# ZhangYizhao/UltraRE

Measured on AMD Instinct MI355X. Metric: training interactions/sec + unlearn retrain wall-time, ml-1m 5-shard SISA, higher is better.
Workload: dtype f32; 1 GPU; ml1m-shaped synthetic 6040x3416, 896914 train rows, 5-shard SISA (uniform grouping), d=32, batch=30000, SGD-momentum-L2, all shards of a rank side by side; parallelism=shards x1, arch=gfx950:sramecc+:xnack-

## Files before the change

ultrare_amd/csrc/perm_chain.hip:

```cpp
#include "ure_internal.h"
#include "mt_jump_dev.h"

namespace ure {
namespace {

constexpr int kMtN = 624, kMtLag = 227;
constexpr int kDrawBlock = 640;
constexpr int kDrawWide = 623;
constexpr int kDrawRing = 8192;
constexpr int64_t kSegmentedRows = 1 << 21;
constexpr int kFewBuckets = 1024;
constexpr int kMaxBuckets = 16384;
constexpr int kTileBlock = 1024;
constexpr int kTileLoads = 4;
constexpr int kTile = kTileBlock * 4 * kTileLoads;
constexpr int kLinkBlock = 512;
constexpr int kLinkLoads = 8;
constexpr int kStage = 6144;
constexpr int kStage10 = 3072, kStage12 = 12288;
constexpr int kStageHeavy = 16384;
constexpr int kHeavyParts = 8;
constexpr int kResolveBlock = 1024;
constexpr int kResolveRows = 4096;
constexpr unsigned kNone = 0xffffffffu;
constexpr unsigned kGoOn = 0x80000000u;
constexpr int64_t kRecordRows = 1 << 20;
constexpr int kRecordShift = 20;
constexpr int kRecordRangeLog2 = 32 - kRecordShift;

__device__ __forceinline__ void lds_barrier()
{
    __builtin_amdgcn_fence(__ATOMIC_RELEASE, "workgroup", "local");
    __builtin_amdgcn_s_barrier();
    __builtin_amdgcn_fence(__ATOMIC_ACQUIRE, "workgroup", "local");
}

__device__ __forceinline__ unsigned mt_temper(unsigned x)
{
    x ^= x >> 11;
    x ^= (x << 7) & 0x9d2c5680u;
    x ^= (x << 15) & 0xefc60000u;
    x ^= x >> 18;
    return x;
}

__device__ __forceinline__ unsigned swap_target(unsigned j, unsigned word, unsigned n) { return j + mt_temper(word) % (n - j); }

template <bool Rec>
struct swap_fmt;
template <>
struct swap_fmt<false> {
    using type = uint2;
    static __device__ __forceinline__ type make(unsigned j, unsigned q, unsigned) { return make_uint2(j, q); }
    static __device__ __forceinline__ type none() { return make_uint2(0u, 0u); }
    static __device__ __forceinline__ unsigned index(type r) { return r.x; }
    static __device__ __forceinline__ unsigned place(type r, unsigned q0) { return r.y - q0; }
};
template <>
struct swap_fmt<true> {
    using type = unsigned;
    static __device__ __forceinline__ type make(unsigned j, unsigned q, unsigned in_range) { return j | (q & in_range) << kRecordShift; }
    static __device__ __forceinline__ type none() { return 0u; }
    static __device__ __forceinline__ unsigned index(type r) { return r & ((1u << kRecordShift) - 1u); }
    static __device__ __forceinline__ unsigned place(type r, unsigned) { return r >> kRecordShift; }
};

struct perm_view {
    unsigned *t, *H, *minv;
    uint2 *pairs;
    unsigned *totals, *cursors, *bases;
};

__host__ __device__ __forceinline__ int64_t words_per_perm(int64_t n_al, int64_t b_al) { return 5 * n_al + 3 * b_al; }

__device__ __forceinline__ perm_view view_of(unsigned *scratch, int perm, int64_t n_al, int64_t b_al)
{
    unsigned *b = scratch + (size_t)perm * (size_t)words_per_perm(n_al, b_al);
    unsigned *c = b + 5 * n_al;
    return perm_view{b, b + n_al, b + 2 * n_al, reinterpret_cast<uint2 *>(b + 3 * n_al), c, c + b_al, c + 2 * b_al};
}

__device__ __forceinline__ unsigned mt_mix(unsigned a, unsigned b)
{
    const unsigned y = (a & 0x80000000u) | (b & 0x7fffffffu);
    return (y >> 1) ^ ((y & 1u) ? 0x9908b0dfu : 0u);
}

__global__ __launch_bounds__(kDrawBlock) void shuffle_seed_kernel(const ure_perm_t *__restrict__ perms, int n_perms, unsigned *__restrict__ states, int J)
{
    const int perm = blockIdx.x, tid = threadIdx.x;
    if (perm >= n_perms) return;
    unsigned *mine = states + (size_t)perm * J * kMtN;
    for (int k = kMtN + tid; k < J * kMtN; k += kDrawBlock) mine[k] = 0u;
    if (tid == 0) {
        unsigned v = (unsigned)((unsigned long long)perms[perm].seed & 0xffffffffull);
        mine[0] = v;
        for (int j = 1; j < kMtN; ++j) {
            v = 1812433253u * (v ^ (v >> 30)) + (unsigned)j;
            mine[j] = v;
        }
    }
}

__global__ __launch_bounds__(kDrawBlock) void shuffle_words_kernel(const ure_perm_t *__restrict__ perms, int n_perms, unsigned *__restrict__ scratch, int64_t n_al,
                                                                   int64_t b_al, int range_log2, const unsigned *__restrict__ states, int J)
{
    constexpr unsigned M = kDrawRing - 1;
    __shared__ unsigned ring[kDrawRing];
    const int tid = threadIdx.x;
    const int perm = blockIdx.x / J, seg = blockIdx.x % J;
    if (perm >= n_perms) return;
    const int n = perms[perm].n;
    if (n <= 0) return;
    const perm_view P = view_of(scratch, perm, n_al, b_al);
    if (seg == 0) {
        const int n_buckets = (int)((((int64_t)n - 1) >> range_log2) + 1);
        for (int b = tid; b < n_buckets; b += kDrawBlock) {
            P.totals[b] = 0u;
            P.cursors[b] = 0u;
        }
    }
    const int64_t w_lo = (int64_t)seg * jmp::kSegWords;
    const int64_t total_all = (int64_t)n - 1;
    if (w_lo >= total_all) return;
    const int total = (int)min<int64_t>(states ? jmp::kSegWords : total_all, total_all - w_lo);
    if (states) {
        const unsigned *blk = states + ((size_t)perm * J + seg) * kMtN;
        for (int k = tid; k < kMtN; k += kDrawBlock) ring[((unsigned)k - kMtN) & M] = blk[k];
    } else if (tid == 0) {
        unsigned v = (unsigned)((unsigned long long)perms[perm].seed & 0xffffffffull);
        ring[(0u - kMtN) & M] = v;
        for (int j = 1; j < kMtN; ++j) {
            v = 1812433253u * (v ^ (v >> 30)) + (unsigned)j;
            ring[((unsigned)j - kMtN) & M] = v;
        }
    }
    __syncthreads();
    unsigned *out = P.t + w_lo;
#pragma unroll 1
    for (int g0 = 0; g0 < total; g0 += kDrawWide) {
        const unsigned g = (unsigned)(g0 + tid);
        if (tid < kDrawWide && (int)g < total) {
            const bool two = g >= (unsigned)kMtLag, three = g >= 2u * kMtLag;
            const unsigned a0 = ring[(g - kMtN) & M], a1 = ring[(g - kMtN + 1) & M];
            const unsigned b0 = ring[(g - kMtLag - kMtN) & M], b1 = ring[(g - kMtLag - kMtN + 1) & M];
            const unsigned c0 = ring[(g - 2 * kMtLag - kMtN) & M], c1 = ring[(g - 2 * kMtLag - kMtN + 1) & M];
            const unsigned x = ring[(g - (three ? 3u * kMtLag : two ? 2u * kMtLag : (unsigned)kMtLag)) & M];
            const unsigned v = x ^ mt_mix(a0, a1) ^ (two ? mt_mix(b0, b1) : 0u) ^ (three ? mt_mix(c0, c1) : 0u);
            ring[g & M] = v;
            out[g] = v;
        }
        lds_barrier();
    }
}

template <int CAP, bool Rec>
__global__ __launch_bounds__(kTileBlock) void shuffle_targets_kernel(const ure_perm_t *__restrict__ perms, int n_perms, int parts_max, unsigned *__restrict__ scratch,
                                                                      int64_t n_al, int64_t b_al, int range_log2, unsigned *__restrict__ mat)
{
    __shared__ unsigned cnt[CAP];
    const int tid = threadIdx.x;
    const int x8 = blockIdx.x & 7, l = blockIdx.x >> 3;
    const int perm = (l / parts_max) * 8 + x8, part = l % parts_max;
    if (perm >= n_perms) return;
    const int n = perms[perm].n;
    const int64_t j0l = (int64_t)part * kTile;
    if (j0l >= (int64_t)n - 1) return;
    const perm_view P = view_of(scratch, perm, n_al, b_al);
    const int n_buckets = (int)((((int64_t)n - 1) >> range_log2) + 1);
    const unsigned j0 = (unsigned)j0l, j_end = (unsigned)(n - 1);
    const int b_lo = (int)(j0 >> range_log2);
    for (int b = b_lo + tid; b < n_buckets; b += kTileBlock) cnt[b] = 0u;
    __syncthreads();
    uint4 *t4 = reinterpret_cast<uint4 *>(P.t);
    uint4 v[kTileLoads];
#pragma unroll
    for (int u = 0; u < kTileLoads; ++u) {
        const unsigned j = j0 + 4u * (unsigned)(tid + u * kTileBlock);
        v[u] = j < j_end ? t4[j >> 2] : make_uint4(0u, 0u, 0u, 0u);
    }
    auto target = [&](unsigned j, unsigned word) {
        if (j >= j_end) return word;
        const unsigned q = swap_target(j, word, (unsigned)n);
        atomicAdd(&cnt[q >> range_log2], 1u);
        return q;
    };
#pragma unroll
    for (int u = 0; u < kTileLoads; ++u) {
        const unsigned j = j0 + 4u * (unsigned)(tid + u * kTileBlock);
        if (j < j_end) {
            v[u].x = target(j, v[u].x);
            v[u].y = target(j + 1, v[u].y);
            v[u].z = target(j + 2, v[u].z);
            v[u].w = target(j + 3, v[u].w);
            if (!Rec) t4[j >> 2] = v[u];
        }
    }
    __syncthreads();
    if (CAP == kFewBuckets) {
        unsigned *row = mat + ((size_t)perm * parts_max + part) * kFewBuckets;
        for (int b = tid; b < n_buckets; b += kTileBlock) row[b] = b >= b_lo ? cnt[b] : 0u;
        return;
    }
    for (int b = b_lo + tid; b < n_buckets; b += kTileBlock) {
        const unsigned c = cnt[b];
        if (c) atomicAdd(&P.totals[b], c);
    }
}

__device__ __forceinline__ bool place_of(int parts_max, int n_perms, int *perm, int *part)
{
    const int x = blockIdx.x & 7, l = blockIdx.x >> 3;
    *perm = (l / parts_max) * 8 + x;
    *part = l % parts_max;
    return *perm < n_perms;
}

template <int Block>
__device__ __forceinline__ unsigned prefix_in_place(unsigned *v, int n, unsigned *wave_sum, unsigned *carry_word)
{
    const int tid = threadIdx.x, lane = tid & 63, wave = tid >> 6;
    if (tid == 0) *carry_word = 0u;
    __syncthreads();
    for (int base = 0; base < n; base += Block) {
        const int x = base + tid;
        const unsigned c = x < n ? v[x] : 0u;
        unsigned s = c;
#pragma unroll
        for (int d = 1; d < 64; d <<= 1) {
            const unsigned o = __shfl_up(s, d, 64);
            if (lane >= d) s += o;
        }
        if (lane == 63) wave_sum[wave] = s;
        __syncthreads();
        unsigned before = *carry_word;
        for (int k = 0; k < wave; ++k) before += wave_sum[k];
        if (x < n) v[x] = before + s - c;
        __syncthreads();
        if (tid == Block - 1) *carry_word = before + s;
    }
    __syncthreads();
    return *carry_word;
}

template <int CAP, bool Rec>
__global__ __launch_bounds__(kTileBlock) void shuffle_bucket_kernel(const ure_perm_t *__restrict__ perms, int n_perms, int parts_max, unsigned *__restrict__ scratch,
                                                                     int64_t n_al, int64_t b_al, int range_log2, const unsigned *__restrict__ mat)
{
    __shared__ unsigned cur[CAP];
    __shared__ unsigned base[CAP];
    __shared__ unsigned wave_sum[kTileBlock / 64];
    __shared__ unsigned s_carry;
    const int tid = threadIdx.x;
    int perm, part;
    if (!place_of(parts_max, n_perms, &perm, &part)) return;
    const int n = perms[perm].n;
    const int64_t j0l = (int64_t)part * kTile;
    if (j0l >= (int64_t)n - 1) {
        if (!(part == 0 && n == 1)) return;
    }
    const perm_view P = view_of(scratch, perm, n_al, b_al);
    const int n_buckets = (int)((((int64_t)n - 1) >> range_log2) + 1);
    const unsigned j0 = (unsigned)j0l, j_end = (unsigned)(n - 1);
    const int b_lo = (int)(j0 >> range_log2);
    const uint4 *t4 = reinterpret_cast<const uint4 *>(P.t);
    uint4 v[kTileLoads];
#pragma unroll
    for (int u = 0; u < kTileLoads; ++u) {
        const unsigned j = j0 + 4u * (unsigned)(tid + u * kTileBlock);
        v[u] = j < j_end ? t4[j >> 2] : make_uint4(0u, 0u, 0u, 0u);
    }
    if (CAP == kFewBuckets) {
        const int n_tiles = (int)(((int64_t)n - 1 + kTile - 1) / kTile);
        const unsigned *m = mat + (size_t)perm * parts_max * kFewBuckets;
        for (int b = tid; b < n_buckets; b += kTileBlock) {
            unsigned all = 0u, before = 0u;
            constexpr int kAtOnce = 8;
            for (int t0 = 0; t0 < n_tiles; t0 += kAtOnce) {
                unsigned c[kAtOnce];
#pragma unroll
                for (int k = 0; k < kAtOnce; ++k) c[k] = m[(size_t)min(t0 + k, n_tiles - 1) * kFewBuckets + b];
#pragma unroll
                for (int k = 0; k < kAtOnce; ++k) {
                    const unsigned ck = t0 + k < n_tiles ? c[k] : 0u;
                    before += t0 + k < part ? ck : 0u;
                    all += ck;
                }
            }
            base[b] = all;
            cur[b] = before;
            if (part == 0) P.totals[b] = all;
        }
        prefix_in_place<kTileBlock>(base, n_buckets, wave_sum, &s_carry);
        for (int b = tid; b < n_buckets; b += kTileBlock) {
            if (part == 0) P.bases[b] = base[b];
            cur[b] += base[b];
        }
        __syncthreads();
    } else {
        for (int b = tid; b < n_buckets; b += kTileBlock) {
            cur[b] = 0u;
            base[b] = P.totals[b];
        }
        __syncthreads();
#pragma unroll
        for (int u = 0; u < kTileLoads; ++u) {
            const unsigned j = j0 + 4u * (unsigned)(tid + u * kTileBlock);
            if (j < j_end) atomicAdd(&cur[v[u].x >> range_log2], 1u);
            if (j + 1 < j_end) atomicAdd(&cur[v[u].y >> range_log2], 1u);
            if (j + 2 < j_end) atomicAdd(&cur[v[u].z >> range_log2], 1u);
            if (j + 3 < j_end) atomicAdd(&cur[v[u].w >> range_log2], 1u);
        }
        prefix_in_place<kTileBlock>(base, n_buckets, wave_sum, &s_carry);
        if (part == 0)
            for (int b = tid; b < n_buckets; b += kTileBlock) P.bases[b] = base[b];
        for (int b = b_lo + tid; b < n_buckets; b += kTileBlock) {
            const unsigned c = cur[b];
            if (c) cur[b] = base[b] + atomicAdd(&P.cursors[b], c);
        }
        __syncthreads();
    }
    static_assert(!Rec || CAP == kFewBuckets, "records: the count matrix's launches only");
    using fmt = swap_fmt<Rec>;
    typename fmt::type *stretches = reinterpret_cast<typename fmt::type *>(P.pairs);
    const unsigned in_range = (1u << range_log2) - 1u;
    auto put = [&](unsigned j, unsigned w) {
        const unsigned q = Rec ? swap_target(j, w, (unsigned)n) : w;
        stretches[atomicAdd(&cur[q >> range_log2], 1u)] = fmt::make(j, q, in_range);
    };
    __builtin_amdgcn_s_waitcnt(0x0F70);
#pragma unroll
    for (int u = 0; u < kTileLoads; ++u) {
        const unsigned j = j0 + 4u * (unsigned)(tid + u * kTileBlock);
        if (j < j_end) put(j, v[u].x);
        if (j + 1 < j_end) put(j + 1, v[u].y);
        if (j + 2 < j_end) put(j + 2, v[u].z);
        if (j + 3 < j_end) put(j + 3, v[u].w);
    }
}

template <int Block, int Per>
__device__ __forceinline__ unsigned prefix_by_lane(unsigned *v, unsigned *wave_sum)
{
    const int tid = threadIdx.x, lane = tid & 63, wave = tid >> 6;
    unsigned c[Per];
    unsigned mine = 0u;
#pragma unroll
    for (int k = 0; k < Per; ++k) {
        c[k] = v[tid * Per + k];
        mine += c[k];
    }
    unsigned s = mine;
#pragma unroll
    for (int d = 1; d < 64; d <<= 1) {
        const unsigned o = __shfl_up(s, d, 64);
        if (lane >= d) s += o;
    }
    if (lane == 63) wave_sum[wave] = s;
    __syncthreads();
    unsigned before = 0u, total = 0u;
#pragma unroll
    for (int k = 0; k < Block / 64; ++k) {
        const unsigned ws = wave_sum[k];
        if (k < wave) before += ws;
        total += ws;
    }
    unsigned run = before + s - mine;
#pragma unroll
    for (int k = 0; k < Per; ++k) {
        v[tid * Per + k] = run;
        run += c[k];
    }
    __syncthreads();
    return total;
}

template <int RL, int Stage, bool Rec>
__global__ __launch_bounds__(kLinkBlock) void shuffle_link_kernel(const ure_perm_t *__restrict__ perms, int n_perms, int parts_max, unsigned *__restrict__ scratch,
                                                                   int64_t n_al, int64_t b_al, int heavy)
{
    static_assert(!Rec || RL <= kRecordRangeLog2, "a record has 12 bits for the target's place in its range");
    using fmt = swap_fmt<Rec>;
    using swap_t = typename fmt::type;
    constexpr int kRange = 1 << RL, kPer = kRange / kLinkBlock;
    __shared__ unsigned off[kRange];
    __shared__ unsigned stage[Stage];
    __shared__ unsigned wave_sum[kLinkBlock / 64];
    const int tid = threadIdx.x;
    int perm, part;
    if (!place_of(parts_max, n_perms, &perm, &part)) return;
    const int n = perms[perm].n;
    const int64_t q0l = (int64_t)part << RL;
    if (q0l >= n) return;
    const int n_buckets = (int)((((int64_t)n - 1) >> RL) + 1);
    if ((part >= n_buckets - kHeavyParts) != (heavy != 0)) return;
    const unsigned q0 = (unsigned)q0l, q1 = (unsigned)min<int64_t>(n, q0l + kRange);
    const int R = (int)(q1 - q0);
    const perm_view P = view_of(scratch, perm, n_al, b_al);
    const unsigned count = P.totals[part], at = P.bases[part];
    const swap_t *mine = reinterpret_cast<const swap_t *>(P.pairs) + at;
#pragma unroll
    for (int k = 0; k < kPer; ++k) off[k * kLinkBlock + tid] = 0u;
    __syncthreads();
    swap_t first[kLinkLoads];
#pragma unroll
    for (int u = 0; u < kLinkLoads; ++u) {
        const unsigned e = (unsigned)(u * kLinkBlock + tid);
        first[u] = e < count ? mine[e] : fmt::none();
    }
#pragma unroll
    for (int u = 0; u < kLinkLoads; ++u)
        if ((unsigned)(u * kLinkBlock + tid) < count) atomicAdd(&off[fmt::place(first[u], q0)], 1u);
    for (unsigned e0 = kLinkBlock * kLinkLoads; e0 < count; e0 += kLinkBlock * kLinkLoads) {
        swap_t m[kLinkLoads];
#pragma unroll
        for (int u = 0; u < kLinkLoads; ++u) {
            const unsigned e = e0 + (unsigned)(u * kLinkBlock + tid);
            m[u] = mine[min(e, count - 1u)];
        }
#pragma unroll
        for (int u = 0; u < kLinkLoads; ++u)
            if (e0 + (unsigned)(u * kLinkBlock + tid) < count) atomicAdd(&off[fmt::place(m[u], q0)], 1u);
    }
    __syncthreads();
    prefix_by_lane<kLinkBlock, kPer>(off, wave_sum);
    const bool in_lds = count <= (unsigned)Stage;
    unsigned *placed = P.t + at;
    auto place = [&](const swap_t m) {
        const unsigned pos = atomicAdd(&off[fmt::place(m, q0)], 1u);
        if (in_lds)
            stage[pos] = fmt::index(m);
        else
            placed[pos] = fmt::index(m);
    };
#pragma unroll
    for (int u = 0; u < kLinkLoads; ++u)
        if ((unsigned)(u * kLinkBlock + tid) < count) place(first[u]);
    for (unsigned e0 = kLinkBlock * kLinkLoads; e0 < count; e0 += kLinkBlock * kLinkLoads) {
        swap_t m[kLinkLoads];
#pragma unroll
        for (int u = 0; u < kLinkLoads; ++u) {
            const unsigned e = e0 + (unsigned)(u * kLinkBlock + tid);
            m[u] = mine[min(e, count - 1u)];
        }
#pragma unroll
        for (int u = 0; u < kLinkLoads; ++u)
            if (e0 + (unsigned)(u * kLinkBlock + tid) < count) place(m[u]);
    }
    if (in_lds) {
        __syncthreads();
    } else {
        __builtin_amdgcn_fence(__ATOMIC_RELEASE, "workgroup");
        __syncthreads();
        __builtin_amdgcn_fence(__ATOMIC_ACQUIRE, "workgroup");
    }
    const unsigned last = (unsigned)(n - 1);
    for (int b0 = 0; b0 < R; b0 += kLinkBlock) {
        unsigned seg0 = 0u;
        bool staged = in_lds;
        if (!in_lds) {
            seg0 = b0 ? off[b0 - 1] : 0u;
            const unsigned seg1 = off[min(b0 + kLinkBlock, R) - 1];
            staged = seg1 - seg0 <= (unsigned)Stage;
            if (staged)
                for (unsigned i = tid; i < seg1 - seg0; i += kLinkBlock) stage[i] = placed[seg0 + i];
            __syncthreads();
        }
        const int x = b0 + tid;
        if (x < R) {
            const unsigned e1 = off[x], e0 = x ? off[x - 1] : 0u;
            const unsigned q = q0 + (unsigned)x;
            auto walk = [&](auto member) {
                unsigned least = kNone;
                for (unsigned i = e0; i < e1; ++i) {
                    const unsigned a = member(i);
                    least = min(least, a);
                    unsigned succ = kNone;
                    for (unsigned m = e0; m < e1; ++m) {
                        const unsigned o = member(m);
                        if (o > a) succ = min(succ, o);
                    }
                    P.H[a] = succ != kNone ? succ : (a == q ? a : (q == last ? last : (kGoOn | q)));
                }
                P.minv[q] = least;
            };
            if (staged)
                walk([&](unsigned i) { return stage[i - seg0]; });
            else
                walk([&](unsigned i) { return placed[i]; });
        }
        if (!in_lds) __syncthreads();
    }
}

__global__ __launch_bounds__(kResolveBlock) void shuffle_resolve_kernel(const ure_perm_t *__restrict__ perms, int n_perms, int parts_max, unsigned *__restrict__ scratch,
                                                                         int64_t n_al, int64_t b_al, unsigned *__restrict__ broken)
{
    int perm, part;
    if (!place_of(parts_max, n_perms, &perm, &part)) return;
    const int n = perms[perm].n;
    const int64_t lo = (int64_t)part * kResolveRows;
    if (lo >= n) return;
    const perm_view P = view_of(scratch, perm, n_al, b_al);
    const unsigned batch = (unsigned)perms[perm].batch;
    uint16_t *out = perms[perm].tags;
    const unsigned hi = (unsigned)min<int64_t>(n, lo + kResolveRows);
    constexpr int U = 4;
    for (unsigned p0 = (unsigned)lo + threadIdx.x; p0 < hi; p0 += U * kResolveBlock) {
        unsigned v[U], h[U];
#pragma unroll
        for (int u = 0; u < U; ++u) {
            const unsigned p = p0 + (unsigned)(u * kResolveBlock);
            v[u] = p < hi ? P.minv[p] : 0u;
            h[u] = p < hi && p != (unsigned)(n - 1) ? P.H[p] : 0u;
        }
#pragma unroll
        for (int u = 0; u < U; ++u) {
            const unsigned p = p0 + (unsigned)(u * kResolveBlock);
            if (p >= hi) continue;
            unsigned r = v[u];
            if (r == kNone) {
                if (p == (unsigned)(n - 1)) {
                    r = p;
                } else {
                    unsigned at = p;
                    r = h[u];
                    while (r & kGoOn) {
                        const unsigned q = r & ~kGoOn;
                        if (q <= at || q >= (unsigned)(n - 1)) {
                            r = kNone;
                            break;
                        }
                        at = q;
                        r = P.H[q];
                    }
                }
            }
            if (r >= (unsigned)n) {
                *broken = 0xdeadu;
                out[p] = (uint16_t)0xFFFFu;
            } else {
                out[p] = (uint16_t)(r / batch);
            }
        }
    }
}

struct link_launch {
    bool records;
    dim3 grid;
    hipStream_t st;
    const ure_perm_t *perms;
    int n_perms, ranges;
    unsigned *scratch;
    int64_t n_al, b_al;
    int heavy;
    template <int RL, int Stage>
    void go() const
    {
        if constexpr (RL <= kRecordRangeLog2) {
            if (records) {
                hipLaunchKernelGGL((shuffle_link_kernel<RL, Stage, true>), grid, dim3(kLinkBlock), 0, st, perms, n_perms, ranges, scratch, n_al, b_al, heavy);
                return;
            }
        }
        hipLaunchKernelGGL((shuffle_link_kernel<RL, Stage, false>), grid, dim3(kLinkBlock), 0, st, perms, n_perms, ranges, scratch, n_al, b_al, heavy);
    }
};

int range_log2_of(int64_t n_max, int32_t wanted)
{
    if (wanted) return wanted;
    return n_max <= ((int64_t)kMaxBuckets << 10) ? 10 : n_max <= ((int64_t)kMaxBuckets << 11) ? 11 : n_max <= ((int64_t)kMaxBuckets << 12) ? 12 : 14;
}

int64_t buckets_al(int64_t n_max, int rl) { return (((n_max - 1) >> rl) + 1 + 63) / 64 * 64; }

}
}

extern "C" int64_t ure_device_shuffle_tags_flag(int64_t n_max, int32_t n_perms)
{
    if (n_max <= 0 || n_perms <= 0) return 0;
    const int64_t n_al = (n_max + 63) / 64 * 64;
    return ure::words_per_perm(n_al, std::min<int64_t>(ure::kMaxBuckets, ure::buckets_al(n_max, 10))) * (int64_t)n_perms;
}

extern "C" int64_t ure_device_shuffle_tags_scratch(int64_t n_max, int32_t n_perms)
{
    if (n_max <= 0 || n_perms <= 0) return 0;
    const int64_t J = n_max > ure::kSegmentedRows ? (n_max - 1 + ure::jmp::kSegWords - 1) / ure::jmp::kSegWords : 0;
    const int64_t tiles = std::max<int64_t>(1, (n_max - 1 + ure::kTile - 1) / ure::kTile);
    return ure_device_shuffle_tags_flag(n_max, n_perms) + 64 + (int64_t)n_perms * J * ure::kMtN + (int64_t)n_perms * tiles * ure::kFewBuckets;
}

extern "C" int ure_device_shuffle_tags(const ure_perm_t *perms, int32_t n_perms, int64_t n_max, uint32_t *scratch, int64_t scratch_words, int32_t range_log2,
                                       void *stream)
{
    using namespace ure;
    URE_ARG(n_perms >= 0 && n_max >= 0 && (range_log2 == 0 || range_log2 == 10 || range_log2 == 11 || range_log2 == 12 || range_log2 == 14));
    if (n_perms == 0 || n_max == 0) return 0;
    URE_ARG(perms && scratch);
    const int rl = range_log2_of(n_max, range_log2);
    if (((n_max - 1) >> rl) + 1 > kMaxBuckets)
        return fail(-1, "ure_device_shuffle_tags: %lld rows: more than %d ranges of %d targets", (long long)n_max, kMaxBuckets, 1 << rl);
    if (scratch_words < ure_device_shuffle_tags_scratch(n_max, n_perms)) return fail(-1, "ure_device_shuffle_tags: scratch too small");
    hipStream_t st = static_cast<hipStream_t>(stream);
    const int64_t n_al = (n_max + 63) / 64 * 64, b_al = buckets_al(n_max, rl);
    uint32_t *broken = scratch + ure_device_shuffle_tags_flag(n_max, n_perms);
    const int64_t slots = ((int64_t)n_perms + 7) / 8;
    const int64_t tiles = std::max<int64_t>(1, (n_max - 1 + kTile - 1) / kTile), ranges = ((n_max - 1) >> rl) + 1, rows = (n_max + kResolveRows - 1) / kResolveRows;
    if (8 * slots * std::max(ranges, rows) > 0x7fffffffll)
        return fail(-1, "ure_device_shuffle_tags: %d permutations of up to %lld rows are too many for one launch", (int)n_perms, (long long)n_max);
    if (n_max > kSegmentedRows) {
        const int64_t J = (n_max - 1 + jmp::kSegWords - 1) / jmp::kSegWords;
        uint32_t *states = broken + 64;
        const uint32_t *levels = nullptr;
        if (jmp::device_levels(jmp::levels_of(J), st, &levels)) return fail(-1, "ure_device_shuffle_tags: the jump polynomials could not be made / uploaded");
        hipLaunchKernelGGL(shuffle_seed_kernel, dim3((unsigned)n_perms), dim3(kDrawBlock), 0, st, perms, (int)n_perms, states, (int)J);
        jmp::launch_tree(states, (int)n_perms, J, levels, st);
        hipLaunchKernelGGL(shuffle_words_kernel, dim3((unsigned)(n_perms * J)), dim3(kDrawBlock), 0, st, perms, (int)n_perms, scratch, n_al, b_al, rl, states, (int)J);
    } else {
        hipLaunchKernelGGL(shuffle_words_kernel, dim3((unsigned)n_perms), dim3(kDrawBlock), 0, st, perms, (int)n_perms, scratch, n_al, b_al, rl,
                           static_cast<const unsigned *>(nullptr), 1);
    }
    const bool few = ranges <= kFewBuckets;
    const int64_t J_all = n_max > kSegmentedRows ? (n_max - 1 + jmp::kSegWords - 1) / jmp::kSegWords : 0;
    uint32_t *mat = broken + 64 + (int64_t)n_perms * J_all * kMtN;
    const bool records = few && n_max <= kRecordRows && rl <= kRecordRangeLog2;
    const dim3 tile_grid((unsigned)(8 * slots * tiles));
    if (records) {
        hipLaunchKernelGGL((shuffle_targets_kernel<kFewBuckets, true>), tile_grid, dim3(kTileBlock), 0, st, perms, (int)n_perms, (int)tiles, scratch, n_al, b_al, rl, mat);
        hipLaunchKernelGGL((shuffle_bucket_kernel<kFewBuckets, true>), tile_grid, dim3(kTileBlock), 0, st, perms, (int)n_perms, (int)tiles, scratch, n_al, b_al, rl, mat);
    } else if (few) {
        hipLaunchKernelGGL((shuffle_targets_kernel<kFewBuckets, false>), tile_grid, dim3(kTileBlock), 0, st, perms, (int)n_perms, (int)tiles, scratch, n_al, b_al, rl, mat);
        hipLaunchKernelGGL((shuffle_bucket_kernel<kFewBuckets, false>), tile_grid, dim3(kTileBlock), 0, st, perms, (int)n_perms, (int)tiles, scratch, n_al, b_al, rl, mat);
    } else {
        hipLaunchKernelGGL((shuffle_targets_kernel<kMaxBuckets, false>), tile_grid, dim3(kTileBlock), 0, st, perms, (int)n_perms, (int)tiles, scratch, n_al, b_al, rl, mat);
        hipLaunchKernelGGL((shuffle_bucket_kernel<kMaxBuckets, false>), tile_grid, dim3(kTileBlock), 0, st, perms, (int)n_perms, (int)tiles, scratch, n_al, b_al, rl, mat);
    }
    for (int heavy = 0; heavy < 2; ++heavy) {
        const link_launch at{records, dim3((unsigned)(8 * slots * ranges)), st, perms, (int)n_perms, (int)ranges, scratch, n_al, b_al, heavy};
        if (rl == 10 && !heavy) at.go<10, kStage10>();
        if (rl == 10 && heavy) at.go<10, kStageHeavy>();
        if (rl == 11 && !heavy) at.go<11, kStage>();
        if (rl == 11 && heavy) at.go<11, kStageHeavy>();
        if (rl == 12 && !heavy) at.go<12, kStage12>();
        if (rl == 12 && heavy) at.go<12, kStageHeavy>();
        if (rl == 14 && !heavy) at.go<14, kStage12>();
        if (rl == 14 && heavy) at.go<14, kStageHeavy>();
    }
    hipLaunchKernelGGL(shuffle_resolve_kernel, dim3((unsigned)(8 * slots * rows)), dim3(kResolveBlock), 0, st, perms, (int)n_perms, (int)rows, scratch, n_al, b_al, broken);
    URE_HIP(hipGetLastError());
    return 0;
}
```

Measured before the change: 7.917 billion interactions/s.

## Streamline MT draw loop with mirrored ring and shrink heavy link grid

The Mersenne-twister word draw now peels the first block so the steady-state loop always XORs three lagged terms. It reads contiguous ring windows through a mirrored head, which avoids per-element masking and branches. Seeding is spread across a wavefront instead of a single thread. The heavy link launch now covers only the last kHeavyParts ranges instead of launching the full range grid and exiting most blocks early. These cut ALU/LDS work in the serial RNG loop and empty-block launch overhead, at the cost of extra LDS for the mirror and more complex indexing.

```diff
diff --git a/ultrare_amd/csrc/perm_chain.hip b/ultrare_amd/csrc/perm_chain.hip
--- a/ultrare_amd/csrc/perm_chain.hip
+++ b/ultrare_amd/csrc/perm_chain.hip
@@ -8,6 +8,10 @@
 constexpr int kDrawBlock = 640;
 constexpr int kDrawWide = 623;
 constexpr int kDrawRing = 8192;
+constexpr int kDrawBack = 2 * kMtLag + kMtN;
+constexpr int kDrawMirror = 512;
+static_assert(kDrawMirror >= 2 * kMtLag + 2, "a lane's window must not wrap");
+static_assert(kDrawRing - kMtN >= kDrawMirror, "the start block lies outside the mirrored head");
 constexpr int64_t kSegmentedRows = 1 << 21;
 constexpr int kFewBuckets = 1024;
 constexpr int kMaxBuckets = 16384;
@@ -106,7 +110,7 @@
                                                                    int64_t b_al, int range_log2, const unsigned *__restrict__ states, int J)
 {
     constexpr unsigned M = kDrawRing - 1;
-    __shared__ unsigned ring[kDrawRing];
+    __shared__ unsigned ring[kDrawRing + kDrawMirror];
     const int tid = threadIdx.x;
     const int perm = blockIdx.x / J, seg = blockIdx.x % J;
     if (perm >= n_perms) return;
@@ -126,30 +130,57 @@
     const int total = (int)min<int64_t>(states ? jmp::kSegWords : total_all, total_all - w_lo);
     if (states) {
         const unsigned *blk = states + ((size_t)perm * J + seg) * kMtN;
-        for (int k = tid; k < kMtN; k += kDrawBlock) ring[((unsigned)k - kMtN) & M] = blk[k];
-    } else if (tid == 0) {
-        unsigned v = (unsigned)((unsigned long long)perms[perm].seed & 0xffffffffull);
-        ring[(0u - kMtN) & M] = v;
-        for (int j = 1; j < kMtN; ++j) {
-            v = 1812433253u * (v ^ (v >> 30)) + (unsigned)j;
-            ring[((unsigned)j - kMtN) & M] = v;
-        }
-    }
-    __syncthreads();
+        for (int k = tid; k < kMtN; k += kDrawBlock) ring[kDrawRing - kMtN + k] = blk[k];
+    } else if (tid < 64) {
+        unsigned v = __builtin_amdgcn_readfirstlane((unsigned)((unsigned long long)perms[perm].seed & 0xffffffffull));
+        constexpr int kAtOnce = 16;
+#pragma unroll 1
+        for (int j0 = 0; j0 < kMtN; j0 += kAtOnce) {
+            unsigned mine = 0u;
+#pragma unroll
+            for (int l = 0; l < kAtOnce; ++l) {
+                if (j0 + l > 0) v = 1812433253u * (v ^ (v >> 30)) + (unsigned)(j0 + l);
+                mine = tid == l ? v : mine;
+            }
+            if (tid < kAtOnce && j0 + tid < kMtN) ring[kDrawRing - kMtN + j0 + tid] = mine;
+        }
+    }
+    __syncthreads();
+    auto keep = [&](unsigned at, unsigned v) {
+        ring[at] = v;
+        if (at < (unsigned)kDrawMirror) ring[kDrawRing + at] = v;
+    };
     unsigned *out = P.t + w_lo;
+    if (tid < kDrawWide && tid < total) {
+        const unsigned g = (unsigned)tid;
+        const bool two = g >= (unsigned)kMtLag, three = g >= 2u * kMtLag;
+        const unsigned a0 = ring[(g - kMtN) & M], a1 = ring[(g - kMtN + 1) & M];
+        const unsigned b0 = ring[(g - kMtLag - kMtN) & M], b1 = ring[(g - kMtLag - kMtN + 1) & M];
+        const unsigned c0 = ring[(g - 2 * kMtLag - kMtN) & M], c1 = ring[(g - 2 * kMtLag - kMtN + 1) & M];
+        const unsigned x = ring[(g - (three ? 3u * kMtLag : two ? 2u * kMtLag : (unsigned)kMtLag)) & M];
+        const unsigned v = x ^ mt_mix(a0 ^ (two ? b0 : 0u) ^ (three ? c0 : 0u), a1 ^ (two ? b1 : 0u) ^ (three ? c1 : 0u));
+        keep(g, v);
+        out[g] = v;
+    }
+    lds_barrier();
+    unsigned rd = (unsigned)(kDrawWide + tid - kDrawBack) & M, wr = (unsigned)(kDrawWide + tid) & M;
+    unsigned *o = out + kDrawWide + tid;
+    int left = tid < kDrawWide ? total - kDrawWide - tid : 0;
 #pragma unroll 1
-    for (int g0 = 0; g0 < total; g0 += kDrawWide) {
-        const unsigned g = (unsigned)(g0 + tid);
-        if (tid < kDrawWide && (int)g < total) {
-            const bool two = g >= (unsigned)kMtLag, three = g >= 2u * kMtLag;
-            const unsigned a0 = ring[(g - kMtN) & M], a1 = ring[(g - kMtN + 1) & M];
-            const unsigned b0 = ring[(g - kMtLag - kMtN) & M], b1 = ring[(g - kMtLag - kMtN + 1) & M];
-            const unsigned c0 = ring[(g - 2 * kMtLag - kMtN) & M], c1 = ring[(g - 2 * kMtLag - kMtN + 1) & M];
-            const unsigned x = ring[(g - (three ? 3u * kMtLag : two ? 2u * kMtLag : (unsigned)kMtLag)) & M];
-            const unsigned v = x ^ mt_mix(a0, a1) ^ (two ? mt_mix(b0, b1) : 0u) ^ (three ? mt_mix(c0, c1) : 0u);
-            ring[g & M] = v;
-            out[g] = v;
-        }
+    for (int g0 = kDrawWide; g0 < total; g0 += kDrawWide) {
+        if (left > 0) {
+            const unsigned *w = ring + rd;
+            const unsigned c0 = w[0], c1 = w[1], b0 = w[kMtLag], b1 = w[kMtLag + 1];
+            const unsigned x = w[kDrawBack - 3 * kMtLag], a0 = w[kDrawBack - kMtN], a1 = w[kDrawBack - kMtN + 1];
+            __builtin_amdgcn_sched_barrier(0);
+            const unsigned v = x ^ mt_mix(a0 ^ b0 ^ c0, a1 ^ b1 ^ c1);
+            keep(wr, v);
+            *o = v;
+        }
+        rd = (rd + (unsigned)kDrawWide) & M;
+        wr = (wr + (unsigned)kDrawWide) & M;
+        o += kDrawWide;
+        left -= kDrawWide;
         lds_barrier();
     }
 }
@@ -390,10 +421,11 @@
     int perm, part;
     if (!place_of(parts_max, n_perms, &perm, &part)) return;
     const int n = perms[perm].n;
+    if (n <= 0) return;
+    const int n_buckets = (int)((((int64_t)n - 1) >> RL) + 1);
+    if (heavy) part += n_buckets - kHeavyParts;
+    if (part < 0 || part >= n_buckets || (part >= n_buckets - kHeavyParts) != (heavy != 0)) return;
     const int64_t q0l = (int64_t)part << RL;
-    if (q0l >= n) return;
-    const int n_buckets = (int)((((int64_t)n - 1) >> RL) + 1);
-    if ((part >= n_buckets - kHeavyParts) != (heavy != 0)) return;
     const unsigned q0 = (unsigned)q0l, q1 = (unsigned)min<int64_t>(n, q0l + kRange);
     const int R = (int)(q1 - q0);
     const perm_view P = view_of(scratch, perm, n_al, b_al);
@@ -551,7 +583,7 @@
     dim3 grid;
     hipStream_t st;
     const ure_perm_t *perms;
-    int n_perms, ranges;
+    int n_perms, parts;
     unsigned *scratch;
     int64_t n_al, b_al;
     int heavy;
@@ -560,11 +592,11 @@
     {
         if constexpr (RL <= kRecordRangeLog2) {
             if (records) {
-                hipLaunchKernelGGL((shuffle_link_kernel<RL, Stage, true>), grid, dim3(kLinkBlock), 0, st, perms, n_perms, ranges, scratch, n_al, b_al, heavy);
+                hipLaunchKernelGGL((shuffle_link_kernel<RL, Stage, true>), grid, dim3(kLinkBlock), 0, st, perms, n_perms, parts, scratch, n_al, b_al, heavy);
                 return;
             }
         }
-        hipLaunchKernelGGL((shuffle_link_kernel<RL, Stage, false>), grid, dim3(kLinkBlock), 0, st, perms, n_perms, ranges, scratch, n_al, b_al, heavy);
+        hipLaunchKernelGGL((shuffle_link_kernel<RL, Stage, false>), grid, dim3(kLinkBlock), 0, st, perms, n_perms, parts, scratch, n_al, b_al, heavy);
     }
 };
 
@@ -610,7 +642,7 @@
     uint32_t *broken = scratch + ure_device_shuffle_tags_flag(n_max, n_perms);
     const int64_t slots = ((int64_t)n_perms + 7) / 8;
     const int64_t tiles = std::max<int64_t>(1, (n_max - 1 + kTile - 1) / kTile), ranges = ((n_max - 1) >> rl) + 1, rows = (n_max + kResolveRows - 1) / kResolveRows;
-    if (8 * slots * std::max(ranges, rows) > 0x7fffffffll)
+    if (8 * slots * std::max<int64_t>({ranges, rows, kHeavyParts}) > 0x7fffffffll)
         return fail(-1, "ure_device_shuffle_tags: %d permutations of up to %lld rows are too many for one launch", (int)n_perms, (long long)n_max);
     if (n_max > kSegmentedRows) {
         const int64_t J = (n_max - 1 + jmp::kSegWords - 1) / jmp::kSegWords;
@@ -640,7 +672,8 @@
         hipLaunchKernelGGL((shuffle_bucket_kernel<kMaxBuckets, false>), tile_grid, dim3(kTileBlock), 0, st, perms, (int)n_perms, (int)tiles, scratch, n_al, b_al, rl, mat);
     }
     for (int heavy = 0; heavy < 2; ++heavy) {
-        const link_launch at{records, dim3((unsigned)(8 * slots * ranges)), st, perms, (int)n_perms, (int)ranges, scratch, n_al, b_al, heavy};
+        const int64_t parts = heavy ? kHeavyParts : ranges;
+        const link_launch at{records, dim3((unsigned)(8 * slots * parts)), st, perms, (int)n_perms, (int)parts, scratch, n_al, b_al, heavy};
         if (rl == 10 && !heavy) at.go<10, kStage10>();
         if (rl == 10 && heavy) at.go<10, kStageHeavy>();
         if (rl == 11 && !heavy) at.go<11, kStage>();
```

Result: faster. 8.219 billion interactions/s, median of 6 (+3.8%).
